# EPFL-VILAB/omnidata

Measured on AMD Instinct MI355X. Metric: images/sec (384x384) DPT-Hybrid surface-normal inference, higher is better.
Workload: dtype bf16; 1 GPU; DPT-Hybrid-384 normal, batch 32/GPU, bf16, 1xMI355X (BASELINE.json configs[1]); batch_per_gpu=32, global_batch=32, parallelism=replicas x1 (no collective in the loop), ranks_seen=1, inflight=1

## Files before the change

### omnidata_amd/csrc/attention.hip

```cpp
#include "common.h"
#include "kernels.h"

namespace dptx {

constexpr int ATT_D = 64;
constexpr int ATT_KT = 64;
constexpr int ATT_K_BYTES = ATT_KT * 128;
constexpr int ATT_V_BYTES = ATT_D * 128;
constexpr int ATT_STAGE = ATT_K_BYTES + ATT_V_BYTES;

__device__ __forceinline__ uint4 lds_read16(const char* p) {
  const u32x4_t v = *(const u32x4_t*)p;
  return uint4{v.x, v.y, v.z, v.w};
}

template <int DT, int PL>
__global__ __launch_bounds__(256, 2) void attention_kernel(const uint16_t* __restrict__ qkv, uint16_t* __restrict__ out,
                                                           int S, int H, int BH, long long plane) {
  extern __shared__ __attribute__((aligned(16))) char smem[];
  constexpr int STAGE = ATT_STAGE * PL;
  const int tid = threadIdx.x, lane = tid & 63, wave = tid >> 6;
  const int lr = lane & 31, lh = lane >> 5;
  const int bh = (int)blockIdx.x % BH, qblk = (int)blockIdx.x / BH;
  const int head = bh % H, b = bh / H;
  const int ld = 3 * H * ATT_D;
  const long long row0 = (long long)b * S;
  const uint16_t* qbase = qkv + head * ATT_D;
  const uint16_t* kbase = qkv + H * ATT_D + head * ATT_D;
  const uint16_t* vbase = qkv + 2 * H * ATT_D + head * ATT_D;

  const int q = qblk * 128 + wave * 32 + lr;
  const int qc = q < S ? q : S - 1;
  const bool wave_active = qblk * 128 + wave * 32 < S;
  uint4 qf[4], ql[4];
#pragma unroll
  for (int ks = 0; ks < 4; ++ks) {
    qf[ks] = *(const uint4*)(qbase + (row0 + qc) * ld + ks * 16 + lh * 8);
    if (PL == 2) ql[ks] = *(const uint4*)(qbase + plane + (row0 + qc) * ld + ks * 16 + lh * 8);
  }

  const u32x4_t zero4 = {0u, 0u, 0u, 0u};
#if defined(__HIP_DEVICE_COMPILE__)
  const int qkv_bytes = (int)((long long)(BH / H) * S * ld * 2);
  const __amdgpu_buffer_rsrc_t rsrc0 = __builtin_amdgcn_make_buffer_rsrc(const_cast<uint16_t*>(qkv), 0, qkv_bytes, 0x00020000);
  const __amdgpu_buffer_rsrc_t rsrc1 = __builtin_amdgcn_make_buffer_rsrc(const_cast<uint16_t*>(qkv) + (PL == 2 ? plane : 0), 0, qkv_bytes, 0x00020000);
  auto dma_kv = [&](int T, int buf) {
#pragma unroll
    for (int pc = 0; pc < 2; ++pc) {
      const int row = (wave * 2 + pc) * 8 + (lane >> 3);
      const int key = 1 + T * ATT_KT + row;
      const bool ok = key < S;
      const unsigned rowoff = (unsigned)((row0 + key) * ld + head * ATT_D);
      const unsigned koff = ok ? (rowoff + H * ATT_D + (((lane & 7) ^ ((row >> 1) & 7)) << 3)) * 2u : 0x80000000u;
      const unsigned voff = ok ? (rowoff + 2 * H * ATT_D + (((lane & 7) ^ (4 * ((row >> 1) & 1))) << 3)) * 2u : 0x80000000u;
      char* dst = smem + buf * STAGE + (wave * 2 + pc) * 1024;
      __builtin_amdgcn_raw_ptr_buffer_load_lds(rsrc0, (__attribute__((address_space(3))) void*)dst, 16, koff, 0, 0, 0);
      __builtin_amdgcn_raw_ptr_buffer_load_lds(rsrc0, (__attribute__((address_space(3))) void*)(dst + ATT_K_BYTES), 16, voff, 0, 0, 0);
      if (PL == 2) {
        __builtin_amdgcn_raw_ptr_buffer_load_lds(rsrc1, (__attribute__((address_space(3))) void*)(dst + ATT_STAGE), 16, koff, 0, 0, 0);
        __builtin_amdgcn_raw_ptr_buffer_load_lds(rsrc1, (__attribute__((address_space(3))) void*)(dst + ATT_STAGE + ATT_K_BYTES), 16, voff, 0, 0, 0);
      }
    }
  };
  const int lq = lane & 15, g16 = (lane >> 4) & 1;
  int va[2];
#pragma unroll
  for (int dt = 0; dt < 2; ++dt)
    va[dt] = (4 * lh + (lq >> 2)) * 128 + (((dt ^ ((lq >> 3) & 1)) * 4 + 2 * g16 + ((lq & 3) >> 1)) << 4) + (lq & 1) * 8;
  typedef short s16x4_t __attribute__((ext_vector_type(4)));
  typedef __attribute__((address_space(3))) s16x4_t* lds_s16x4_p;
  auto read_vt = [&](const char* vtile, int dt, int i) -> uint4 {
    const __attribute__((address_space(3))) char* vb = (const __attribute__((address_space(3))) char*)vtile + va[dt] + i * 2048;
    const s16x4_t r0_ = __builtin_amdgcn_ds_read_tr16_b64_v4i16((lds_s16x4_p)vb);
    const s16x4_t r1_ = __builtin_amdgcn_ds_read_tr16_b64_v4i16((lds_s16x4_p)(vb + 1024));
    const uint2 u0 = __builtin_bit_cast(uint2, r0_), u1 = __builtin_bit_cast(uint2, r1_);
    return uint4{u0.x, u0.y, u1.x, u1.y};
  };
#else
  auto dma_kv = [&](int, int) {};
  auto read_vt = [&](const char*, int, int) -> uint4 { return uint4{0u, 0u, 0u, 0u}; };
#endif

  const int ntiles = (S - 1 + ATT_KT - 1) / ATT_KT;
  if (ntiles > 0) dma_kv(0, 0);

  const float cexp = 0.125f * 1.4426950408889634f;
  f32x16_t o[2];
  float m_run, l_run;
  {
    float part = 0.f;
#pragma unroll
    for (int ks = 0; ks < 4; ++ks) {
      float qv[8], kv[8];
      u32x4_t qh = {qf[ks].x, qf[ks].y, qf[ks].z, qf[ks].w}, qlo = zero4;
      if (PL == 2) qlo = u32x4_t{ql[ks].x, ql[ks].y, ql[ks].z, ql[ks].w};
      unpack8x<DT, PL>(qh, qlo, qv);
      const u32x4_t kh = *(const u32x4_t*)(kbase + row0 * ld + ks * 16 + lh * 8);
      u32x4_t klo = zero4;
      if (PL == 2) klo = *(const u32x4_t*)(kbase + plane + row0 * ld + ks * 16 + lh * 8);
      unpack8x<DT, PL>(kh, klo, kv);
#pragma unroll
      for (int e = 0; e < 8; ++e) part = fmaf(qv[e], kv[e], part);
    }
    m_run = part + __shfl_xor(part, 32, 64);
    l_run = lh == 0 ? 1.f : 0.f;
#pragma unroll
    for (int dt = 0; dt < 2; ++dt)
#pragma unroll
      for (int g = 0; g < 4; ++g) {
        const int d = dt * 32 + 8 * g + 4 * lh;
        const uint2 vh = *(const uint2*)(vbase + row0 * ld + d);
        float v4[4] = {T16<DT>::tof((uint16_t)(vh.x & 0xffffu)), T16<DT>::tof((uint16_t)(vh.x >> 16)),
                       T16<DT>::tof((uint16_t)(vh.y & 0xffffu)), T16<DT>::tof((uint16_t)(vh.y >> 16))};
        if (PL == 2) {
          const uint2 vl = *(const uint2*)(vbase + plane + row0 * ld + d);
          v4[0] += T16<DT>::tof((uint16_t)(vl.x & 0xffffu)); v4[1] += T16<DT>::tof((uint16_t)(vl.x >> 16));
          v4[2] += T16<DT>::tof((uint16_t)(vl.y & 0xffffu)); v4[3] += T16<DT>::tof((uint16_t)(vl.y >> 16));
        }
#pragma unroll
        for (int e = 0; e < 4; ++e) o[dt][4 * g + e] = v4[e];
      }
  }

  asm volatile("s_waitcnt vmcnt(0)" ::: "memory");
  __syncthreads();
  for (int t = 0; t < ntiles; ++t) {
    const bool more = (t + 1) < ntiles;
    if (more) dma_kv(t + 1, (t + 1) & 1);
    const char* sk = smem + (t & 1) * STAGE;
    const char* sv = sk + ATT_K_BYTES;
    if (wave_active) {
      f32x16_t s0, s1;
#pragma unroll
      for (int r = 0; r < 16; ++r) { s0[r] = 0.f; s1[r] = 0.f; }
#pragma unroll
      for (int ks = 0; ks < 4; ++ks) {
        const int chunk = 2 * ks + lh;
        const int koff0 = lr * 128 + ((chunk ^ ((lr >> 1) & 7)) << 4);
        const int koff1 = koff0 + 32 * 128;
        const uint4 kf0 = lds_read16(sk + koff0), kf1 = lds_read16(sk + koff1);
        if (PL == 2) {
          const uint4 kl0 = lds_read16(sk + ATT_STAGE + koff0), kl1 = lds_read16(sk + ATT_STAGE + koff1);
          s0 = T16<DT>::mfma32(kl0, qf[ks], s0);
          s1 = T16<DT>::mfma32(kl1, qf[ks], s1);
          s0 = T16<DT>::mfma32(kf0, ql[ks], s0);
          s1 = T16<DT>::mfma32(kf1, ql[ks], s1);
        }
        s0 = T16<DT>::mfma32(kf0, qf[ks], s0);
        s1 = T16<DT>::mfma32(kf1, qf[ks], s1);
      }
      const int key0 = 1 + t * ATT_KT + 4 * lh;
      if (key0 + 32 + 28 + 3 >= S) {
#pragma unroll
        for (int r = 0; r < 16; ++r) {
          if (key0 + (r & 3) + 8 * (r >> 2) >= S) s0[r] = -1e30f;
          if (key0 + 32 + (r & 3) + 8 * (r >> 2) >= S) s1[r] = -1e30f;
        }
      }
      float mx = s0[0], mx1 = s1[0];
#pragma unroll
      for (int r = 1; r < 16; ++r) { mx = fmaxf(mx, s0[r]); mx1 = fmaxf(mx1, s1[r]); }
      mx = fmaxf(mx, mx1);
      mx = fmaxf(mx, __shfl_xor(mx, 32, 64));
      const float m_new = fmaxf(m_run, mx);
      const float alpha = __builtin_amdgcn_exp2f((m_run - m_new) * cexp);
      const bool grew = m_new > m_run;
      m_run = m_new;
      const float mc = m_new * cexp;
      float pv0[16], pv1[16];
      float ps = 0.f;
#pragma unroll
      for (int r = 0; r < 16; ++r) {
        pv0[r] = __builtin_amdgcn_exp2f(fmaf(s0[r], cexp, -mc));
        pv1[r] = __builtin_amdgcn_exp2f(fmaf(s1[r], cexp, -mc));
        ps += pv0[r] + pv1[r];
      }
      l_run = l_run * alpha + ps;
      if (__any(grew)) {
#pragma unroll
        for (int r = 0; r < 16; ++r) { o[0][r] *= alpha; o[1][r] *= alpha; }
      }
      uint4 pf[4], pl2[4];
      pf[0] = pack8<DT>(pv0);
      pf[1] = pack8<DT>(pv0 + 8);
      pf[2] = pack8<DT>(pv1);
      pf[3] = pack8<DT>(pv1 + 8);
      if (PL == 2) {
        float ph[8];
#pragma unroll
        for (int i = 0; i < 4; ++i) {
          const float* src = (i < 2 ? pv0 : pv1) + (i & 1) * 8;
          unpack8<DT>(pf[i], ph);
#pragma unroll
          for (int r = 0; r < 8; ++r) ph[r] = src[r] - ph[r];
          pl2[i] = pack8<DT>(ph);
        }
      }
#pragma unroll
      for (int i = 0; i < 4; ++i) {
#pragma unroll
        for (int dt = 0; dt < 2; ++dt) {
          const uint4 vf = read_vt(sv, dt, i);
          if (PL == 2) {
            const uint4 vl = read_vt(sv + ATT_STAGE, dt, i);
            o[dt] = T16<DT>::mfma32(vl, pf[i], o[dt]);
            o[dt] = T16<DT>::mfma32(vf, pl2[i], o[dt]);
          }
          o[dt] = T16<DT>::mfma32(vf, pf[i], o[dt]);
        }
      }
    }
    asm volatile("s_waitcnt vmcnt(0)" ::: "memory");
    __syncthreads();
  }

  const float l_tot = l_run + __shfl_xor(l_run, 32, 64);
  const float inv = 1.0f / l_tot;
  if (q < S) {
    uint16_t* op = out + (row0 + q) * (long long)(H * ATT_D) + head * ATT_D;
#pragma unroll
    for (int dt = 0; dt < 2; ++dt)
#pragma unroll
      for (int g = 0; g < 4; ++g) {
        const float v0 = o[dt][4 * g] * inv, v1 = o[dt][4 * g + 1] * inv, v2 = o[dt][4 * g + 2] * inv, v3 = o[dt][4 * g + 3] * inv;
        uint2 w;
        w.x = T16<DT>::pack2(v0, v1);
        w.y = T16<DT>::pack2(v2, v3);
        *(uint2*)(op + dt * 32 + 8 * g + 4 * lh) = w;
        if (PL == 2) {
          uint2 l;
          l.x = T16<DT>::pack2(v0 - T16<DT>::tof((uint16_t)(w.x & 0xffffu)), v1 - T16<DT>::tof((uint16_t)(w.x >> 16)));
          l.y = T16<DT>::pack2(v2 - T16<DT>::tof((uint16_t)(w.y & 0xffffu)), v3 - T16<DT>::tof((uint16_t)(w.y >> 16)));
          *(uint2*)(op + plane + dt * 32 + 8 * g + 4 * lh) = l;
        }
      }
  }
}

hipError_t launch_attention(int mode, const void* qkv, void* out, int B, int S, int heads, Planes pl, hipStream_t stream) {
  const int BH = B * heads;
  if ((long long)B * S * 3 * heads * ATT_D * 2 >= (1ll << 31)) return hipErrorInvalidValue;
  dim3 grid(((S + 127) / 128) * BH);
  if (mode == MODE_BF16)
    hipLaunchKernelGGL((attention_kernel<DT_BF16, 1>), grid, dim3(256), 2 * ATT_STAGE, stream, (const uint16_t*)qkv, (uint16_t*)out, S, heads, BH, 0ll);
  else if (mode == MODE_FP16)
    hipLaunchKernelGGL((attention_kernel<DT_FP16, 1>), grid, dim3(256), 2 * ATT_STAGE, stream, (const uint16_t*)qkv, (uint16_t*)out, S, heads, BH, 0ll);
  else if (mode == MODE_BF16X3) {
    ensure_dyn_smem((const void*)attention_kernel<DT_BF16, 2>, 4 * ATT_STAGE);
    hipLaunchKernelGGL((attention_kernel<DT_BF16, 2>), grid, dim3(256), 4 * ATT_STAGE, stream, (const uint16_t*)qkv, (uint16_t*)out, S, heads, BH, pl.act);
  } else if (mode == MODE_FP16X3) {
    ensure_dyn_smem((const void*)attention_kernel<DT_FP16, 2>, 4 * ATT_STAGE);
    hipLaunchKernelGGL((attention_kernel<DT_FP16, 2>), grid, dim3(256), 4 * ATT_STAGE, stream, (const uint16_t*)qkv, (uint16_t*)out, S, heads, BH, pl.act);
  } else
    return hipErrorInvalidValue;
  return hipGetLastError();
}

}
```

### omnidata_amd/build.py

```python
from __future__ import annotations

import os
import subprocess
import sys

HERE = os.path.dirname(os.path.abspath(__file__))
CSRC = os.path.join(HERE, "csrc")
LIB = os.path.join(HERE, "libdptx.so")
SOURCES = ["gemm.hip", "gemm_fp16.hip", "gemm_fp16e.hip", "gemm_x3.hip", "gemm_x2.hip", "gemm_fp8.hip", "attention.hip", "norm.hip", "misc.hip", "stem.hip", "head.hip", "prepost.hip", "refocus.hip", "midas_loss.hip", "vnl_loss.hip", "normal_loss.hip", "eval_metrics.hip", "engine.hip", "ops.hip"]
HEADERS = ["common.h", "kernels.h", "gemm_impl.h", "select.h", os.path.join("..", "..", "include", "dptx.h")]
_NOPK = ["-Xclang", "-target-feature", "-Xclang", "-packed-fp32-ops"]
SOURCE_FLAGS = {src: list(_NOPK) for src in ("norm.hip", "misc.hip", "gemm.hip", "gemm_fp16.hip", "gemm_fp16e.hip", "gemm_x3.hip",
                                             "gemm_x2.hip", "gemm_fp8.hip", "refocus.hip",
                                             "midas_loss.hip", "vnl_loss.hip", "normal_loss.hip", "eval_metrics.hip")}
EXPERIMENT_HEADERS = []


def source_hash(extra_flags=()) -> str:
    import hashlib
    h = hashlib.sha256()
    for name in sorted(SOURCES + HEADERS + EXPERIMENT_HEADERS):
        path = os.path.join(CSRC, name)
        h.update(os.path.basename(name).encode() + b"\0")
        with open(path, "rb") as f:
            h.update(f.read())
    h.update(" ".join(extra_flags).encode())
    h.update(repr(sorted(SOURCE_FLAGS.items())).encode())
    return h.hexdigest()[:16]


def _newer(dst: str, srcs) -> bool:
    if not os.path.exists(dst):
        return False
    t = os.path.getmtime(dst)
    return all(os.path.getmtime(s) <= t for s in srcs)


def built_hash(suffix: str = "") -> str:
    path = os.path.join(CSRC, "build" + suffix, "engine.srchash")
    return open(path).read().strip() if os.path.exists(path) else ""


def build(force: bool = False, verbose: bool = False) -> str:
    import fcntl
    suffix = os.environ.get("DPTX_LIB_SUFFIX", "")
    objdir = os.path.join(CSRC, "build" + suffix)
    os.makedirs(objdir, exist_ok=True)
    with open(os.path.join(objdir, ".lock"), "w") as lock:
        fcntl.flock(lock, fcntl.LOCK_EX)
        try:
            return _build_locked(force, verbose, suffix, objdir)
        finally:
            fcntl.flock(lock, fcntl.LOCK_UN)


def _build_locked(force: bool, verbose: bool, suffix: str, objdir: str) -> str:
    hipcc = os.environ.get("HIPCC", "/opt/rocm/bin/hipcc")
    extra = os.environ.get("DPTX_CXXFLAGS", "").split()
    LIB = os.path.join(HERE, f"libdptx{suffix}.so")
    hdrs = [os.path.join(CSRC, h) for h in HEADERS + EXPERIMENT_HEADERS]
    src_hash = source_hash(extra)
    hash_file = os.path.join(objdir, "engine.srchash")
    old_hash = open(hash_file).read().strip() if os.path.exists(hash_file) else ""
    objs = []
    procs = []
    for src in SOURCES:
# ... 38 lines not shown
```

### omnidata_amd/csrc/gemm.hip

```cpp
#include "gemm_impl.h"

namespace dptx {

hipError_t launch_gemm_16(int dt, const GemmParams& p, hipStream_t stream) {
  return dt == DT_BF16 ? launch_dt<DT_BF16, 1>(p, stream) : launch_gemm_fp16(p, stream);
}

void gemm_params_dense(GemmParams& p, int M, int N, int K) {
  p = GemmParams{};
  p.M = M; p.N = N; p.K = K; p.ldw = K;
  p.a_rpi = M > 0 ? M : 1; p.Wout = p.a_rpi; p.Hin = 1; p.Win = p.a_rpi; p.Cin = K; p.a_pix_stride = K;
  p.a_img_stride = 0; p.a_off = 0; p.ksz = 1; p.stride = 1; p.pad_t = 0; p.pad_l = 0;
  p.c_rpi = 0x7fffffff; p.c_img_rows = 0; p.c_row_off = 0; p.ldc = N;
  p.a_bytes = (long long)M * K * 2;
}

void gemm_params_conv(GemmParams& p, int B, int Hin, int Win, int Cin, int Cout, int ksz, int stride, int pad_t, int pad_l,
                      int Hout, int Wout, int a_elem_bytes) {
  p = GemmParams{};
  p.M = B * Hout * Wout; p.N = Cout; p.K = ksz * ksz * Cin; p.ldw = p.K;
  p.a_rpi = Hout * Wout; p.Wout = Wout; p.Hin = Hin; p.Win = Win; p.Cin = Cin; p.a_pix_stride = Cin;
  p.a_img_stride = (long long)Hin * Win * Cin; p.a_off = 0; p.ksz = ksz; p.stride = stride; p.pad_t = pad_t; p.pad_l = pad_l;
  p.c_rpi = 0x7fffffff; p.c_img_rows = 0; p.c_row_off = 0; p.ldc = Cout;
  p.a_bytes = (long long)B * Hin * Win * Cin * a_elem_bytes;
  p.k_tap_fast = (ksz == 3 && Cin >= 512) ? 1 : 0;
}

static thread_local long long* g_trace = nullptr;
void gemm_set_trace(long long* dev_buf) { g_trace = dev_buf; }
static thread_local int g_debug_flags = 0;
void gemm_set_debug_flags(int flags) { g_debug_flags = flags; }
static thread_local float g_cu_share = 1.0f;
void gemm_set_cu_share(float share) { g_cu_share = share > 0.f && share <= 1.f ? share : 1.0f; }

hipError_t launch_gemm(int mode, const GemmParams& p0, hipStream_t stream) {
  GemmParams p = p0;
  p.trace = g_trace;
  p.debug_flags = g_debug_flags;
  if (p.cu_share <= 0.f) p.cu_share = g_cu_share;
  p.a_rpi_rcp = 1.0f / (float)(p.a_rpi > 0 ? p.a_rpi : 1);
  p.wout_rcp = 1.0f / (float)(p.Wout > 0 ? p.Wout : 1);
  if (p.gn_part != nullptr && (p.gn_hw % 32 != 0 || p.N % 32 != 0 || p.gn_cpg != p.N / 32 || p.gn_cpg < 2 || p.gn_cpg > 32 ||
                               (p.gn_cpg & (p.gn_cpg - 1)) != 0 || p.bias != nullptr || p.act != 0))
    return hipErrorInvalidValue;
  if (p.row_stats != nullptr && (p.N % 128 != 0 || p.stats_nblk != 8 || p.N / 128 > 8)) return hipErrorInvalidValue;
  if (p.ln_stats != nullptr && (p.R1 != nullptr || p.R2 != nullptr || p.bias_per_img || p.ln_colsum == nullptr || (p.ln_nblk != 6 && p.ln_nblk != 8) ||
                                p.c_rpi != 0x7fffffff || p.gn_part != nullptr))
    return hipErrorInvalidValue;
  if (mode == MODE_FP8) {
    if (p.K % 128 != 0 || p.Cin % 128 != 0 || p.M <= 0 || p.N % 32 != 0 || p.ldw < p.K || p.ldw % 16 != 0 || p.gn_part != nullptr)
      return hipErrorInvalidValue;
    return launch_gemm_fp8(p, stream);
  }
  if (p.K % BK != 0 || p.Cin % BK != 0 || p.M <= 0 || p.N % 32 != 0 || p.ldw < p.K || p.ldw % 8 != 0) return hipErrorInvalidValue;
  if (mode == MODE_BF16) return p.epi2 ? hipErrorInvalidValue : launch_gemm_16(DT_BF16, p, stream);
  if (mode == MODE_FP16) return p.epi2 ? launch_gemm_fp16e(p, stream) : launch_gemm_16(DT_FP16, p, stream);
  if (mode == MODE_BF16X3) return launch_gemm_x3(DT_BF16, p, stream);
  if (mode == MODE_FP16X3) return p.a_hi_only ? launch_gemm_x2(p, stream) : launch_gemm_x3(DT_FP16, p, stream);
  return hipErrorInvalidValue;
}

}
```

### omnidata_amd/csrc/gemm_impl.h

```cpp
#pragma once
#include <cstdlib>
#include <type_traits>

#include "common.h"
#include "kernels.h"

namespace dptx {

constexpr int BK = 64;

__device__ __forceinline__ int row_div(int m, int d, float rcp, bool big, int& rem) {
  if (big) {
    const int q = m / d;
    rem = m - q * d;
    return q;
  }
  int q = (int)((float)m * rcp);
  int r = m - q * d;
  if (r < 0) { --q; r += d; }
  if (r >= d) { ++q; r -= d; }
  rem = r;
  return q;
}

// ... 66 lines not shown
#pragma unroll
      for (int ks = 0; ks < HK; ++ks) {
#pragma unroll
        for (int i = 0; i < TM; ++i) {
          if (RELU_A) af[ks][i] = relu8(af[ks][i]);
#pragma unroll
          for (int j = 0; j < TN; ++j) acc[i][j] = T16<DT>::mfma32(af[ks][i], bf[ks][j], acc[i][j]);
        }
      }
      if (HK != BK / 16) __builtin_amdgcn_sched_barrier(0);
    }
    return;
  } else {
    u32x4_t af[2][TM], bf[2][TN], al[2][TM], bl[2][TN];
    auto read = [&](int s_, int ks) {
      const int chunk = 2 * ks + lh;
#pragma unroll
      for (int i = 0; i < TM; ++i) {
        const int row = wm * (TM * 32) + i * 32 + lr;
        const int off = row * 128 + ((chunk ^ ((row >> 1) & 7)) << 4);
        af[s_][i] = *(const u32x4_t*)(sa + off);
        if (XT == 3) al[s_][i] = *(const u32x4_t*)(sa + a_lo + off);
      }
#pragma unroll
      for (int j = 0; j < TN; ++j) {
        const int row = wn * (TN * 32) + j * 32 + lr;
        const int off = row * 128 + ((chunk ^ ((row >> 1) & 7)) << 4);
        bf[s_][j] = *(const u32x4_t*)(sb + off);
        bl[s_][j] = *(const u32x4_t*)(sb + b_lo + off);
      }
    };
    auto mma = [&](int s_) {
#pragma unroll
      for (int i = 0; i < TM; ++i) {
        if (RELU_A) {
          if (XT == 3) relu8_planes(af[s_][i], al[s_][i]);
          else af[s_][i] = relu8(af[s_][i]);
        }
#pragma unroll
        for (int j = 0; j < TN; ++j) {
          if (XT == 3) acc[i][j] = T16<DT>::mfma32(al[s_][i], bf[s_][j], acc[i][j]);
          acc[i][j] = T16<DT>::mfma32(af[s_][i], bl[s_][j], acc[i][j]);
          acc[i][j] = T16<DT>::mfma32(af[s_][i], bf[s_][j], acc[i][j]);
        }
      }
    };
    read(0, 0);
#pragma unroll
    for (int ks = 0; ks < BK / 16; ++ks) {
      if (ks + 1 < BK / 16) read((ks + 1) & 1, ks + 1);
      __builtin_amdgcn_sched_barrier(0);
      mma(ks & 1);
      __builtin_amdgcn_sched_barrier(0);
    }
  }
}

template <int DT, int BM, int BN, int TM, int TN, int PL = 1, int NT = 256, int SLABS = 1, bool WP = false>
__device__ __forceinline__ void epilogue(const GemmParams& p, char* smem, int m0, int n0, int wm, int wn, int lr, int lh,
                                         int tid, f32x16_t (&acc)[TM][TN], int row_pitch = 0, bool dma_in_flight = false,
                                         int trace_row = -1, const char* lds_ln = nullptr) {
  static_assert(SLABS == 1 || SLABS == TM, "one slab, or one per MFMA row tile");
  static_assert(!WP || (SLABS == TM && TN == 2), "wave-private staging: one 32 x 64 block per wave and slab");
  constexpr int CT_PITCH = WP ? 72 : BN + 4;
  constexpr int CT_ROWS = WP ? 32 : BM / SLABS;
  constexpr int NCH = WP ? 8 : BN / 8;
  constexpr int RPP = WP ? 8 : NT / NCH;
  constexpr int ITER = CT_ROWS / RPP;
  constexpr int WAVES_N = BN / (TN * 32);
  static_assert(CT_ROWS % RPP == 0, "rows per pass must divide the slab");
#ifdef DPTX_TRACE
#define DPTX_ESTAMP(SLOT)                                                                                          \
  do {                                                                                                             \
    if (p.trace != nullptr && blockIdx.x == 0 && tid == 0 && trace_row >= 0)                                       \
      p.trace[(48 + trace_row) * 4 + (SLOT)] = (long long)__builtin_readcyclecounter();                            \
  } while (0)
#else
#define DPTX_ESTAMP(SLOT) do { } while (0)
  (void)trace_row;
#endif
  DPTX_ESTAMP(0);
  float* ct = (float*)smem + (WP ? (wm * WAVES_N + wn) * (32 * CT_PITCH) : 0);
  const int cn = WP ? tid & 7 : tid % NCH;
  const int rr = WP ? (tid & 63) >> 3 : tid / NCH;
  const int n = n0 + (WP ? wn * (TN * 32) : 0) + cn * 8;

  if (p.gn_part != nullptr) {
    const int cpg = p.gn_cpg;
    const int cpg_sh = __builtin_ctz(cpg);
    int gn_hw = p.gn_hw;
    asm volatile("" : "+s"(gn_hw));
#pragma unroll
    for (int i = 0; i < TM; ++i) {
      const int mb = m0 + (wm * TM + i) * 32;
      const int img = mb / gn_hw;
      const int blk = (mb - img * gn_hw) >> 5;
#pragma unroll
      for (int j = 0; j < TN; ++j) {
        float sm = 0.f, sq = 0.f;
#pragma unroll
        for (int r = 0; r < 16; ++r) { const float v = acc[i][j][r]; sm += v; sq = fmaf(v, v, sq); }
        sm += __shfl_xor(sm, 32, 64);
        sq += __shfl_xor(sq, 32, 64);
        for (int o = 1; o < cpg; o <<= 1) { sm += __shfl_xor(sm, o, 64); sq += __shfl_xor(sq, o, 64); }
        if (lh == 0 && (lr & (cpg - 1)) == 0 && mb < p.M) {
          const int g = (n0 + (wn * TN + j) * 32 + lr) >> cpg_sh;
          float2* dst = (float2*)p.gn_part + ((long long)img * p.gn_blocks + blk) * 32 + g;
          *dst = make_float2(sm, sq);
        }
      }
    }
  }

  float bias_c[8];
#pragma unroll
  for (int e = 0; e < 8; ++e) bias_c[e] = 0.f;
  if (p.bias != nullptr && !p.bias_per_img) {
    const float4 b0 = *(const float4*)(p.bias + n), b1 = *(const float4*)(p.bias + n + 4);
    bias_c[0] = b0.x; bias_c[1] = b0.y; bias_c[2] = b0.z; bias_c[3] = b0.w;
    bias_c[4] = b1.x; bias_c[5] = b1.y; bias_c[6] = b1.z; bias_c[7] = b1.w;
  }
  float osc[8];
  if (p.out_scale != 0.f) {
#pragma unroll
    for (int e = 0; e < 8; ++e) osc[e] = p.out_scale;
    if (p.out_scale_v != nullptr) {
      const float4 s0 = *(const float4*)(p.out_scale_v + n), s1 = *(const float4*)(p.out_scale_v + n + 4);
      osc[0] *= s0.x; osc[1] *= s0.y; osc[2] *= s0.z; osc[3] *= s0.w;
      osc[4] *= s1.x; osc[5] *= s1.y; osc[6] *= s1.z; osc[7] *= s1.w;
    }
  }
  const bool remap = p.c_rpi != 0x7fffffff;
  int c_rpi = p.c_rpi;
  asm volatile("" : "+s"(c_rpi));
  float2* lnrow = (float2*)(smem + (WP ? (size_t)(NT / 64) * 32 * CT_PITCH * 4 : (size_t)CT_ROWS * CT_PITCH * 4));
  if (p.ln_stats != nullptr) {
    const bool all8 = p.ln_nblk == 8;
    for (int r = tid; r < BM; r += NT) {
      int R = r;
      if (row_pitch) R = (R >> 5) * row_pitch + (R & 31);
      int m = m0 + R;
      m = m < p.M ? m : m0;
      const float4* st = lds_ln != nullptr ? (const float4*)(lds_ln + r * 64) : (const float4*)(p.ln_stats + (long long)m * 16);
      const float4 r0 = st[0], r1_ = st[1], r2_ = st[2], r3_ = st[3];
      const float sm = (r0.x + r0.z) + (r1_.x + r1_.z) + ((r2_.x + r2_.z) + (all8 ? r3_.x + r3_.z : 0.f));
      const float sq = (r0.y + r0.w) + (r1_.y + r1_.w) + ((r2_.y + r2_.w) + (all8 ? r3_.y + r3_.w : 0.f));
      lnrow[r] = ln_mu_rstd(sm, sq, p.ln_inv_dim, p.ln_eps);
    }
    if (WP) __syncthreads();
  }
  DPTX_ESTAMP(1);
  constexpr int GR_ = SLABS > 1 ? 2 : (ITER < 4 ? ITER : 4);
  static_assert(ITER % GR_ == 0, "row groups");

  auto body = [&](auto r1m_, auto r2m_, auto bpi_, auto lnf_) {
    constexpr int R1M = decltype(r1m_)::value, R2M = decltype(r2m_)::value, BPI = decltype(bpi_)::value;
    constexpr bool LNF = decltype(lnf_)::value != 0;
    constexpr int GR = (SLABS > 1 && (R1M < 0 || (PL == 2 && R1M != 0 && R2M != 0))) ? 1 : GR_;
    constexpr int NGR = ITER / GR;
    float ln_c[8];
    if (LNF) {
      const float4 c0 = *(const float4*)(p.ln_colsum + n), c1 = *(const float4*)(p.ln_colsum + n + 4);
      ln_c[0] = c0.x; ln_c[1] = c0.y; ln_c[2] = c0.z; ln_c[3] = c0.w;
      ln_c[4] = c1.x; ln_c[5] = c1.y; ln_c[6] = c1.z; ln_c[7] = c1.w;
    }
// ... 1219 lines not shown
```

### omnidata_amd/csrc/kernels.h

```cpp
#pragma once
#include <hip/hip_runtime.h>
#include <stdint.h>

#include "common.h"

namespace dptx {

void ensure_dyn_smem(const void* kernel, size_t bytes);

struct GemmParams {
  const void* A;
  const void* W;
  void* C;
  const float* bias;
  const void* R1;
  const void* R2;
  int M, N, K;
  int ldw;
  int a_rpi, Wout, Hin, Win, Cin, a_pix_stride;
  long long a_img_stride, a_off;
  long long a_bytes;
  int ksz, stride, pad_t, pad_l;
  int c_rpi, c_img_rows, c_row_off, ldc;
  int r2_bcast;
  int bias_per_img;
  int act;
  int a_relu;
  int a_fp32;
  int c_fp32, r1_fp32, r2_fp32;
  Planes planes;
  int epi2, c_hi_only, r1_hi_only, r2_hi_only;
  int a_hi_only;
  int xcd_m, xcd_n;
  float cu_share;
  float pad0;
  int k_tap_fast;
  float* gn_part;
  int gn_hw, gn_blocks, gn_cpg;
  void* C8;
  int q_relu;
  float out_scale, q_scale;
  const float* out_scale_v;
  void* C16;
  float* row_stats;
  int stats_nblk;
  const float* ln_stats;
  const float* ln_colsum;
  int ln_nblk;
  float ln_eps, ln_inv_dim;
  long long* trace;
  int debug_flags;
  float a_rpi_rcp, wout_rcp;
};

void gemm_params_dense(GemmParams& p, int M, int N, int K);
void gemm_params_conv(GemmParams& p, int B, int Hin, int Win, int Cin, int Cout, int ksz, int stride, int pad_t, int pad_l,
                      int Hout, int Wout, int a_elem_bytes);
hipError_t launch_gemm(int dtype, const GemmParams& p, hipStream_t stream);
void gemm_set_trace(long long* dev_buf);
void gemm_set_debug_flags(int flags);
void gemm_set_cu_share(float share);

hipError_t launch_attention(int mode, const void* qkv, void* out, int B, int S, int heads, Planes pl, hipStream_t stream);

hipError_t launch_layernorm(int mode, const float* x, const float* gamma, const float* beta, void* y,
                            int M, int C, float eps, Planes pl, hipStream_t stream);

struct GnParams {
  const void* X; void* Y;
  const float* gamma; const float* beta;
  float* partial;
  const void* R;
  const float* r_gamma; const float* r_beta; const float* r_partial;
  int B, HW, C, relu;
  float eps;
  int nrec;
};
int gn_chunks(int HW, int C);
hipError_t launch_gn_stats(int mode, const void* X, float* partial, int B, int HW, int C, Planes pl, hipStream_t stream);
hipError_t launch_gn_apply(int mode, const GnParams& p, Planes pl, hipStream_t stream);
hipError_t launch_gn_relu_maxpool(int mode, const void* X, void* Y, const float* gamma, const float* beta,
                                  const float* partial, int B, int H, int W, int C, float eps, Planes pl, hipStream_t stream);

hipError_t launch_stem_conv(int mode, const void* x, int io, const void* Wt, void* y, int B, int H, int W, Planes pl,
                            hipStream_t stream);

hipError_t launch_upsample2x(int mode, const void* X, void* Y, int B, int H, int W, int C, Planes pl, hipStream_t stream,
                             void* Y8 = nullptr, float q_scale = 1.0f, bool out_hi_only = false);
hipError_t launch_amax(int mode, const void* X, size_t n, int relu, unsigned* amax_bits, hipStream_t stream);

hipError_t launch_nonfinite_scan(int mode, const void* X, size_t n, unsigned* flag, hipStream_t stream);

hipError_t launch_checksum(const void* p, size_t bytes, unsigned long long* out, hipStream_t stream);
hipError_t launch_spin(long long ticks_100mhz, hipStream_t stream);

hipError_t launch_head_out(int mode, const void* X, const float* w, const float* b, void* y, int io, int B, int HW,
                           int Cout, int relu, Planes pl, hipStream_t stream);

hipError_t launch_head_tail(int mode, const void* H0, const void* W2, const float* b2, const float* w4, const float* b4,
                            void* y, int io, int B, int Hs, int Ws, int C, int relu_out, hipStream_t stream, Planes pl = Planes{0, 0});
hipError_t launch_pos_resize(const float* src, float* dst, int g_old, int gh, int gw, int C, hipStream_t stream);
hipError_t launch_cls_rows(int mode, const float* cls, const float* pos, float* X, int B, int S, int C, void* X16, float* stats,
                           hipStream_t stream, void* X8 = nullptr, float q_scale = 1.0f);

hipError_t launch_readout_cls(int mode, const float* x, long long x_stride, const void* W, int ldw, int w_off,
                              const float* bias, float* out, int B, int N, int K, Planes pl, hipStream_t stream, int x16 = 0);
hipError_t launch_cast_f32(int mode, const float* src, void* dst, size_t n, Planes pl, hipStream_t stream);

hipError_t launch_patchify16(int mode, const void* x, int io, void* P, int B, int H, int W, Planes pl, hipStream_t stream);
hipError_t launch_depth_to_space(int mode, const void* G, void* Y, int B, int h, int w, int k, int C, Planes pl, hipStream_t stream);

hipError_t launch_to_f32(int mode, const void* src, float* dst, size_t n, Planes pl, hipStream_t stream);

// ... 2 lines not shown
```

Before: 2678 images/s.

## Remap attention blocks by head groups, hoist DMA offsets, use permlane32 swaps

Changes the block-to-(head,qblock) mapping so consecutive blocks cover groups of 8 heads across all query blocks, which improves K/V reuse in L2. Per-lane K/V buffer offsets are precomputed once and the tile offset is passed through soffset, which removes address arithmetic from the loop. Cross-half reductions use permlane32_swap instead of shuffles. The output epilogue swaps halves so each lane writes 16-byte stores instead of 8-byte ones. The grid is padded to a multiple of 8 heads with an early exit, and the unsigned 32-bit soffset math relies on the existing size guard.

Result: no change. 2691 images/s (median of 6 runs) (+0.5%).

```diff
diff --git a/omnidata_amd/csrc/attention.hip b/omnidata_amd/csrc/attention.hip
--- a/omnidata_amd/csrc/attention.hip
+++ b/omnidata_amd/csrc/attention.hip
@@ -9,19 +9,48 @@
 constexpr int ATT_V_BYTES = ATT_D * 128;
 constexpr int ATT_STAGE = ATT_K_BYTES + ATT_V_BYTES;
 
+__device__ __forceinline__ void swap_halves(unsigned& a, unsigned& b) {
+#if defined(__HIP_DEVICE_COMPILE__)
+  const auto r = __builtin_amdgcn_permlane32_swap(a, b, false, false);
+  a = r[0];
+  b = r[1];
+#endif
+}
+__device__ __forceinline__ float max_both_halves(float x) {
+  unsigned a = __float_as_uint(x), b = a;
+  swap_halves(a, b);
+  return fmaxf(__uint_as_float(a), __uint_as_float(b));
+}
+
+__device__ __forceinline__ float sum_both_halves(float x) {
+  unsigned a = __float_as_uint(x), b = a;
+  swap_halves(a, b);
+  return __uint_as_float(a) + __uint_as_float(b);
+}
+
 __device__ __forceinline__ uint4 lds_read16(const char* p) {
   const u32x4_t v = *(const u32x4_t*)p;
   return uint4{v.x, v.y, v.z, v.w};
 }
+
+__host__ __device__ __forceinline__ void att_block_map(int id, int nq, int& pair, int& qblk) {
+  const int j = id >> 3;
+  pair = (j / nq) * 8 + (id & 7);
+  qblk = j % nq;
+}
+inline int att_grid(int S, int BH) { return 8 * ((BH + 7) / 8) * ((S + 127) / 128); }
 
 template <int DT, int PL>
 __global__ __launch_bounds__(256, 2) void attention_kernel(const uint16_t* __restrict__ qkv, uint16_t* __restrict__ out,
                                                            int S, int H, int BH, long long plane) {
   extern __shared__ __attribute__((aligned(16))) char smem[];
   constexpr int STAGE = ATT_STAGE * PL;
-  const int tid = threadIdx.x, lane = tid & 63, wave = tid >> 6;
+  const int tid = threadIdx.x, lane = tid & 63;
+  const int wave = __builtin_amdgcn_readfirstlane(tid >> 6);
   const int lr = lane & 31, lh = lane >> 5;
-  const int bh = (int)blockIdx.x % BH, qblk = (int)blockIdx.x / BH;
+  int bh, qblk;
+  att_block_map((int)blockIdx.x, (S + 127) >> 7, bh, qblk);
+  if (bh >= BH) return;
   const int head = bh % H, b = bh / H;
   const int ld = 3 * H * ATT_D;
   const long long row0 = (long long)b * S;
@@ -44,21 +73,29 @@
   const int qkv_bytes = (int)((long long)(BH / H) * S * ld * 2);
   const __amdgpu_buffer_rsrc_t rsrc0 = __builtin_amdgcn_make_buffer_rsrc(const_cast<uint16_t*>(qkv), 0, qkv_bytes, 0x00020000);
   const __amdgpu_buffer_rsrc_t rsrc1 = __builtin_amdgcn_make_buffer_rsrc(const_cast<uint16_t*>(qkv) + (PL == 2 ? plane : 0), 0, qkv_bytes, 0x00020000);
+  unsigned koff0[2], voff0[2];
+  int krow[2];
+#pragma unroll
+  for (int pc = 0; pc < 2; ++pc) {
+    const int row = (wave * 2 + pc) * 8 + (lane >> 3);
+    const unsigned rowoff = (unsigned)((row0 + 1 + row) * ld + head * ATT_D);
+    krow[pc] = row;
+    koff0[pc] = (rowoff + H * ATT_D + (((lane & 7) ^ ((row >> 1) & 7)) << 3)) * 2u;
+    voff0[pc] = (rowoff + 2 * H * ATT_D + (((lane & 7) ^ (4 * ((row >> 1) & 1))) << 3)) * 2u;
+  }
   auto dma_kv = [&](int T, int buf) {
+    const int soff = T * ATT_KT * ld * 2;
+    const int left = S - 1 - T * ATT_KT;
 #pragma unroll
     for (int pc = 0; pc < 2; ++pc) {
-      const int row = (wave * 2 + pc) * 8 + (lane >> 3);
-      const int key = 1 + T * ATT_KT + row;
-      const bool ok = key < S;
-      const unsigned rowoff = (unsigned)((row0 + key) * ld + head * ATT_D);
-      const unsigned koff = ok ? (rowoff + H * ATT_D + (((lane & 7) ^ ((row >> 1) & 7)) << 3)) * 2u : 0x80000000u;
-      const unsigned voff = ok ? (rowoff + 2 * H * ATT_D + (((lane & 7) ^ (4 * ((row >> 1) & 1))) << 3)) * 2u : 0x80000000u;
+      const bool ok = krow[pc] < left;
+      const unsigned koff = ok ? koff0[pc] : 0x80000000u, voff = ok ? voff0[pc] : 0x80000000u;
       char* dst = smem + buf * STAGE + (wave * 2 + pc) * 1024;
-      __builtin_amdgcn_raw_ptr_buffer_load_lds(rsrc0, (__attribute__((address_space(3))) void*)dst, 16, koff, 0, 0, 0);
-      __builtin_amdgcn_raw_ptr_buffer_load_lds(rsrc0, (__attribute__((address_space(3))) void*)(dst + ATT_K_BYTES), 16, voff, 0, 0, 0);
+      __builtin_amdgcn_raw_ptr_buffer_load_lds(rsrc0, (__attribute__((address_space(3))) void*)dst, 16, koff, soff, 0, 0);
+      __builtin_amdgcn_raw_ptr_buffer_load_lds(rsrc0, (__attribute__((address_space(3))) void*)(dst + ATT_K_BYTES), 16, voff, soff, 0, 0);
       if (PL == 2) {
-        __builtin_amdgcn_raw_ptr_buffer_load_lds(rsrc1, (__attribute__((address_space(3))) void*)(dst + ATT_STAGE), 16, koff, 0, 0, 0);
-        __builtin_amdgcn_raw_ptr_buffer_load_lds(rsrc1, (__attribute__((address_space(3))) void*)(dst + ATT_STAGE + ATT_K_BYTES), 16, voff, 0, 0, 0);
+        __builtin_amdgcn_raw_ptr_buffer_load_lds(rsrc1, (__attribute__((address_space(3))) void*)(dst + ATT_STAGE), 16, koff, soff, 0, 0);
+        __builtin_amdgcn_raw_ptr_buffer_load_lds(rsrc1, (__attribute__((address_space(3))) void*)(dst + ATT_STAGE + ATT_K_BYTES), 16, voff, soff, 0, 0);
       }
     }
   };
@@ -102,7 +139,7 @@
 #pragma unroll
       for (int e = 0; e < 8; ++e) part = fmaf(qv[e], kv[e], part);
     }
-    m_run = part + __shfl_xor(part, 32, 64);
+    m_run = sum_both_halves(part);
     l_run = lh == 0 ? 1.f : 0.f;
 #pragma unroll
     for (int dt = 0; dt < 2; ++dt)
@@ -161,7 +198,7 @@
 #pragma unroll
       for (int r = 1; r < 16; ++r) { mx = fmaxf(mx, s0[r]); mx1 = fmaxf(mx1, s1[r]); }
       mx = fmaxf(mx, mx1);
-      mx = fmaxf(mx, __shfl_xor(mx, 32, 64));
+      mx = max_both_halves(mx);
       const float m_new = fmaxf(m_run, mx);
       const float alpha = __builtin_amdgcn_exp2f((m_run - m_new) * cexp);
       const bool grew = m_new > m_run;
@@ -214,33 +251,48 @@
     __syncthreads();
   }
 
-  const float l_tot = l_run + __shfl_xor(l_run, 32, 64);
+  const float l_tot = sum_both_halves(l_run);
   const float inv = 1.0f / l_tot;
+  uint4 sth[4], stl[4];
+#pragma unroll
+  for (int dt = 0; dt < 2; ++dt)
+#pragma unroll
+    for (int g = 0; g < 4; g += 2) {
+      uint2 w[2], l[2];
+#pragma unroll
+      for (int j = 0; j < 2; ++j) {
+        const int r = 4 * (g + j);
+        const float v0 = o[dt][r] * inv, v1 = o[dt][r + 1] * inv, v2 = o[dt][r + 2] * inv, v3 = o[dt][r + 3] * inv;
+        w[j].x = T16<DT>::pack2(v0, v1);
+        w[j].y = T16<DT>::pack2(v2, v3);
+        if (PL == 2) {
+          l[j].x = T16<DT>::pack2(v0 - T16<DT>::tof((uint16_t)(w[j].x & 0xffffu)), v1 - T16<DT>::tof((uint16_t)(w[j].x >> 16)));
+          l[j].y = T16<DT>::pack2(v2 - T16<DT>::tof((uint16_t)(w[j].y & 0xffffu)), v3 - T16<DT>::tof((uint16_t)(w[j].y >> 16)));
+        }
+      }
+      swap_halves(w[0].x, w[1].x);
+      swap_halves(w[0].y, w[1].y);
+      sth[dt * 2 + g / 2] = uint4{w[0].x, w[0].y, w[1].x, w[1].y};
+      if (PL == 2) {
+        swap_halves(l[0].x, l[1].x);
+        swap_halves(l[0].y, l[1].y);
+        stl[dt * 2 + g / 2] = uint4{l[0].x, l[0].y, l[1].x, l[1].y};
+      }
+    }
   if (q < S) {
-    uint16_t* op = out + (row0 + q) * (long long)(H * ATT_D) + head * ATT_D;
-#pragma unroll
-    for (int dt = 0; dt < 2; ++dt)
-#pragma unroll
-      for (int g = 0; g < 4; ++g) {
-        const float v0 = o[dt][4 * g] * inv, v1 = o[dt][4 * g + 1] * inv, v2 = o[dt][4 * g + 2] * inv, v3 = o[dt][4 * g + 3] * inv;
-        uint2 w;
-        w.x = T16<DT>::pack2(v0, v1);
-        w.y = T16<DT>::pack2(v2, v3);
-        *(uint2*)(op + dt * 32 + 8 * g + 4 * lh) = w;
-        if (PL == 2) {
-          uint2 l;
-          l.x = T16<DT>::pack2(v0 - T16<DT>::tof((uint16_t)(w.x & 0xffffu)), v1 - T16<DT>::tof((uint16_t)(w.x >> 16)));
-          l.y = T16<DT>::pack2(v2 - T16<DT>::tof((uint16_t)(w.y & 0xffffu)), v3 - T16<DT>::tof((uint16_t)(w.y >> 16)));
-          *(uint2*)(op + plane + dt * 32 + 8 * g + 4 * lh) = l;
-        }
-      }
+    uint16_t* op = out + (row0 + q) * (long long)(H * ATT_D) + head * ATT_D + 8 * lh;
+#pragma unroll
+    for (int i = 0; i < 4; ++i) {
+      *(uint4*)(op + 16 * i) = sth[i];
+      if (PL == 2) *(uint4*)(op + plane + 16 * i) = stl[i];
+    }
   }
 }
 
 hipError_t launch_attention(int mode, const void* qkv, void* out, int B, int S, int heads, Planes pl, hipStream_t stream) {
   const int BH = B * heads;
   if ((long long)B * S * 3 * heads * ATT_D * 2 >= (1ll << 31)) return hipErrorInvalidValue;
-  dim3 grid(((S + 127) / 128) * BH);
+  dim3 grid(att_grid(S, BH));
   if (mode == MODE_BF16)
     hipLaunchKernelGGL((attention_kernel<DT_BF16, 1>), grid, dim3(256), 2 * ATT_STAGE, stream, (const uint16_t*)qkv, (uint16_t*)out, S, heads, BH, 0ll);
   else if (mode == MODE_FP16)
```

## Add persistent weight-resident kernel for small-K 1x1 convolutions

Applied to the files above, without the earlier changes.

Adds a specialized streaming kernel for 1x1 convs with K of 64/128/256. It keeps the whole weight panel resident in LDS, gives each wave its own 32-row A tiles with prefetch, and stages output through LDS for coalesced stores. It is routed in automatically for a whitelist of shapes in the ResNet backbone of DPT-Hybrid. The aim is to cut the per-tile weight reloads and K-loop overhead that the generic GEMM pays on these thin-K convolutions. The GN stats epilogue is factored into a shared helper so the new kernel can reuse it.

Result: faster. 2616 images/s before, 2658 images/s after (median of 6 runs) (+1.6%).

```diff
diff --git a/omnidata_amd/build.py b/omnidata_amd/build.py
--- a/omnidata_amd/build.py
+++ b/omnidata_amd/build.py
@@ -7,11 +7,11 @@
 HERE = os.path.dirname(os.path.abspath(__file__))
 CSRC = os.path.join(HERE, "csrc")
 LIB = os.path.join(HERE, "libdptx.so")
-SOURCES = ["gemm.hip", "gemm_fp16.hip", "gemm_fp16e.hip", "gemm_x3.hip", "gemm_x2.hip", "gemm_fp8.hip", "attention.hip", "norm.hip", "misc.hip", "stem.hip", "head.hip", "prepost.hip", "refocus.hip", "midas_loss.hip", "vnl_loss.hip", "normal_loss.hip", "eval_metrics.hip", "engine.hip", "ops.hip"]
+SOURCES = ["gemm.hip", "gemm_fp16.hip", "gemm_fp16e.hip", "gemm_x3.hip", "gemm_x2.hip", "gemm_fp8.hip", "conv1x1.hip", "attention.hip", "norm.hip", "misc.hip", "stem.hip", "head.hip", "prepost.hip", "refocus.hip", "midas_loss.hip", "vnl_loss.hip", "normal_loss.hip", "eval_metrics.hip", "engine.hip", "ops.hip"]
 HEADERS = ["common.h", "kernels.h", "gemm_impl.h", "select.h", os.path.join("..", "..", "include", "dptx.h")]
 _NOPK = ["-Xclang", "-target-feature", "-Xclang", "-packed-fp32-ops"]
 SOURCE_FLAGS = {src: list(_NOPK) for src in ("norm.hip", "misc.hip", "gemm.hip", "gemm_fp16.hip", "gemm_fp16e.hip", "gemm_x3.hip",
-                                             "gemm_x2.hip", "gemm_fp8.hip", "refocus.hip",
+                                             "gemm_x2.hip", "gemm_fp8.hip", "conv1x1.hip", "refocus.hip",
                                              "midas_loss.hip", "vnl_loss.hip", "normal_loss.hip", "eval_metrics.hip")}
 EXPERIMENT_HEADERS = []
 
diff --git a/omnidata_amd/csrc/conv1x1.hip b/omnidata_amd/csrc/conv1x1.hip
--- /dev/null
+++ b/omnidata_amd/csrc/conv1x1.hip
@@ -0,0 +1,209 @@
+#include "gemm_impl.h"
+
+namespace dptx {
+
+constexpr int C1_STG_PITCH = 144;
+constexpr int C1_STG_WAVE = 16 * C1_STG_PITCH;
+constexpr int C1_WAVES = 4;
+
+template <int KT, int BN>
+constexpr size_t conv1x1_smem_bytes() {
+  return (size_t)KT * BN * 128 + (size_t)C1_WAVES * KT * 32 * 128 + (size_t)C1_WAVES * C1_STG_WAVE;
+}
+
+template <int DT, int KT, int BN>
+__global__ __launch_bounds__(64 * C1_WAVES, KT <= 2 ? 2 : 1) void conv1x1_stream_kernel(const GemmParams p) {
+#if defined(__HIP_DEVICE_COMPILE__)
+  constexpr int NSUB = BN / 64;
+  constexpr int KS = KT * 4;
+  constexpr int W_BYTES = KT * BN * 128;
+  constexpr int A_WAVE = KT * 32 * 128;
+  extern __shared__ __attribute__((aligned(16))) char smem[];
+
+  const int tid = threadIdx.x;
+  const int lane = tid & 63;
+  const int wave = __builtin_amdgcn_readfirstlane(tid >> 6);
+  const int lr = lane & 31, lh = lane >> 5;
+
+  const int npan = p.N / BN;
+  const int x = (int)blockIdx.x & 7, l = (int)blockIdx.x >> 3;
+  const int n0 = (l % npan) * BN;
+  const int slots = ((int)gridDim.x / npan) * C1_WAVES;
+  const int rb_total = (p.M + 31) >> 5;
+  int rb = ((l / npan) * 8 + x) * C1_WAVES + wave;
+
+  const int w_bytes = (int)((long long)p.N * p.ldw * 2);
+  const __amdgpu_buffer_rsrc_t rsrcA = __builtin_amdgcn_make_buffer_rsrc(const_cast<void*>(p.A), 0, (int)p.a_bytes, 0x00020000);
+  const __amdgpu_buffer_rsrc_t rsrcW = __builtin_amdgcn_make_buffer_rsrc(const_cast<void*>(p.W), 0, w_bytes, 0x00020000);
+
+  char* const sw = smem;
+  char* const sa = smem + W_BYTES + wave * A_WAVE;
+  char* const stg = smem + W_BYTES + C1_WAVES * A_WAVE + wave * C1_STG_WAVE;
+
+  const int kc = lane & 7, r0 = lane >> 3;
+  auto issue_a = [&](int rblk) {
+#pragma unroll
+    for (int i = 0; i < 4; ++i) {
+      const int row = r0 + 8 * i;
+      const int m = rblk * 32 + row;
+      const bool ok = m < p.M;
+      const int mm = ok ? m : 0;
+      int rem, ox;
+      const int img = row_div(mm, p.a_rpi, p.a_rpi_rcp, false, rem);
+      const int oy = row_div(rem, p.Wout, p.wout_rcp, false, ox);
+      const int iy = oy * p.stride - p.pad_t, ix = ox * p.stride - p.pad_l;
+      const bool valid = ok && ((unsigned)iy < (unsigned)p.Hin) && ((unsigned)ix < (unsigned)p.Win);
+      const long long e = (long long)img * p.a_img_stride + p.a_off + ((long long)iy * p.Win + ix) * p.a_pix_stride +
+                          (kc ^ ((row >> 1) & 7)) * 8;
+      const unsigned base = (unsigned)(e * 2);
+#pragma unroll
+      for (int kt = 0; kt < KT; ++kt) {
+        const unsigned vo = valid ? base + kt * 128 : OOB;
+        __builtin_amdgcn_raw_ptr_buffer_load_lds(rsrcA, (__attribute__((address_space(3))) void*)(sa + kt * 4096 + i * 1024), 16, vo,
+                                                 0, 0, 0);
+      }
+    }
+  };
+
+  if (rb < rb_total) issue_a(rb);
+  for (int idx = wave; idx < KT * (BN / 8); idx += C1_WAVES) {
+    const int kt = idx / (BN / 8), rg = idx - kt * (BN / 8);
+    const int row = rg * 8 + r0;
+    const unsigned vo = (unsigned)(((long long)(n0 + row) * p.ldw + kt * 64 + (kc ^ ((row >> 1) & 7)) * 8) * 2);
+    __builtin_amdgcn_raw_ptr_buffer_load_lds(rsrcW, (__attribute__((address_space(3))) void*)(sw + kt * (BN * 128) + rg * 1024), 16, vo,
+                                             0, 0, 0);
+  }
+  float bias_c[NSUB][2];
+#pragma unroll
+  for (int s = 0; s < NSUB; ++s)
+#pragma unroll
+    for (int j = 0; j < 2; ++j) bias_c[s][j] = p.bias != nullptr ? p.bias[n0 + s * 64 + j * 32 + lr] : 0.f;
+  asm volatile("s_waitcnt vmcnt(0)" ::: "memory");
+  __syncthreads();
+
+  const int swz = (lr >> 1) & 7;
+  const unsigned sel = (lr & 1) ? 0x03020706u : 0x05040100u;
+  const int cn = lane & 7, rr = lane >> 3;
+
+  for (; rb < rb_total; rb += slots) {
+    const int m0 = rb * 32;
+    u32x4_t af[KS];
+#pragma unroll
+    for (int ks = 0; ks < KS; ++ks)
+      af[ks] = *(const u32x4_t*)(sa + (ks >> 2) * 4096 + lr * 128 + (((2 * (ks & 3) + lh) ^ swz) << 4));
+    asm volatile("s_waitcnt lgkmcnt(0)" ::: "memory");
+    const bool prefetch = rb + slots < rb_total;
+    if (prefetch) issue_a(rb + slots);
+
+#pragma unroll
+    for (int s = 0; s < NSUB; ++s) {
+      f32x16_t acc[1][2];
+#pragma unroll
+      for (int j = 0; j < 2; ++j)
+#pragma unroll
+        for (int r = 0; r < 16; ++r) acc[0][j][r] = 0.f;
+#pragma unroll
+      for (int kt = 0; kt < KT; ++kt) {
+        u32x4_t bf[4][2];
+#pragma unroll
+        for (int q = 0; q < 4; ++q)
+#pragma unroll
+          for (int j = 0; j < 2; ++j)
+            bf[q][j] = *(const u32x4_t*)(sw + kt * (BN * 128) + (s * 64 + j * 32 + lr) * 128 + (((2 * q + lh) ^ swz) << 4));
+        __builtin_amdgcn_sched_barrier(0);
+#pragma unroll
+        for (int q = 0; q < 4; ++q)
+#pragma unroll
+          for (int j = 0; j < 2; ++j) acc[0][j] = T16<DT>::mfma32(af[kt * 4 + q], bf[q][j], acc[0][j]);
+      }
+      if (s == 0) {
+        __builtin_amdgcn_sched_barrier(0);
+        asm volatile("s_waitcnt vmcnt(0)" ::: "memory");
+      }
+      if (p.gn_part != nullptr) gn_records<1, 2>(p, m0, n0 + s * 64, 0, 0, lr, lh, acc);
+
+#pragma unroll
+      for (int h = 0; h < 2; ++h) {
+        asm volatile("" ::: "memory");
+        __builtin_amdgcn_wave_barrier();
+#pragma unroll
+        for (int j = 0; j < 2; ++j)
+#pragma unroll
+          for (int t = 0; t < 4; ++t) {
+            float v0 = acc[0][j][8 * h + 2 * t] + bias_c[s][j], v1 = acc[0][j][8 * h + 2 * t + 1] + bias_c[s][j];
+            if (p.act == 1) { v0 = fmaxf(v0, 0.f); v1 = fmaxf(v1, 0.f); }
+            const uint32_t own = T16<DT>::pack2(v0, v1);
+            const uint32_t nb = (uint32_t)__builtin_amdgcn_update_dpp(0, (int)own, 0xB1, 0xf, 0xf, false);
+            const uint32_t o = __builtin_amdgcn_perm(nb, own, sel);
+            const int rl = ((2 * t) & 3) + (lr & 1) + 8 * (t >> 1) + 4 * lh;
+            *(uint32_t*)(stg + rl * C1_STG_PITCH + (j * 32 + (lr & ~1)) * 2) = o;
+          }
+        asm volatile("" ::: "memory");
+        __builtin_amdgcn_wave_barrier();
+#pragma unroll
+        for (int pp = 0; pp < 2; ++pp) {
+          const int rl = rr + 8 * pp;
+          const u32x4_t d = *(const u32x4_t*)(stg + rl * C1_STG_PITCH + cn * 16);
+          const int m = m0 + 16 * h + rl;
+          if (m < p.M) *(u32x4_t*)((uint16_t*)p.C + (long long)(p.c_row_off + m) * p.ldc + (n0 + s * 64 + cn * 8)) = d;
+        }
+      }
+    }
+  }
+#endif
+}
+
+bool conv1x1_stream_eligible(int mode, const GemmParams& p) {
+  if (mode != MODE_BF16 && mode != MODE_FP16) return false;
+  if (p.ksz != 1 || p.pad_t != 0 || p.pad_l != 0 || (p.stride != 1 && p.stride != 2)) return false;
+  if (p.K != p.Cin || (p.K != 64 && p.K != 128 && p.K != 256) || p.N % 64 != 0) return false;
+  if (p.a_fp32 || p.c_fp32 || p.epi2 || p.a_relu || p.R1 != nullptr || p.R2 != nullptr || p.bias_per_img) return false;
+  if (p.c_rpi != 0x7fffffff || p.C8 != nullptr || p.C16 != nullptr || p.out_scale != 0.f) return false;
+  if (p.row_stats != nullptr || p.ln_stats != nullptr || (p.act != 0 && p.act != 1)) return false;
+  if (p.ldc % 8 != 0 || p.a_pix_stride % 8 != 0 || p.a_off % 8 != 0 || p.a_img_stride % 8 != 0) return false;
+  if (p.a_bytes <= 0 || p.a_bytes >= (1ll << 31) || (long long)p.N * p.ldw * 2 >= (1ll << 31) || p.M >= (1 << 23)) return false;
+  return true;
+}
+
+bool conv1x1_stream_adopted(const GemmParams& p) {
+  if (p.stride != 1) return false;
+  if (p.K == 64) return p.N == 256 || p.N == 64;
+  if (p.K == 128) return p.N == 512;
+  if (p.K == 256) return p.N == 64 || p.N == 128 || (p.N == 256 && p.a_rpi >= 48 * 48);
+  return false;
+}
+
+template <int DT, int KT, int BN>
+static hipError_t launch_c1(const GemmParams& p, hipStream_t stream) {
+  constexpr size_t smem = conv1x1_smem_bytes<KT, BN>();
+  static_assert(smem <= 160 * 1024 && (KT > 2 || 2 * smem <= 160 * 1024), "two blocks per CU at K <= 128");
+  const int npan = p.N / BN;
+  const int rb_total = (p.M + 31) / 32;
+  const int want = (rb_total + C1_WAVES - 1) / C1_WAVES;
+  int cap = (KT <= 2 ? 512 : 256) / npan;
+  if (cap < 8) cap = 8;
+  int groups = want < cap ? want : cap;
+  groups = (groups + 7) / 8 * 8;
+  auto k = conv1x1_stream_kernel<DT, KT, BN>;
+  set_smem_attr(k, smem);
+  hipLaunchKernelGGL(k, dim3(groups * npan), dim3(64 * C1_WAVES), smem, stream, p);
+  return hipGetLastError();
+}
+
+template <int DT>
+static hipError_t launch_c1_dt(const GemmParams& p, hipStream_t stream) {
+  if (p.K == 64) {
+    if (p.N % 256 == 0) return launch_c1<DT, 1, 256>(p, stream);
+    if (p.N % 128 == 0) return launch_c1<DT, 1, 128>(p, stream);
+    return launch_c1<DT, 1, 64>(p, stream);
+  }
+  if (p.K == 128) return p.N % 128 == 0 ? launch_c1<DT, 2, 128>(p, stream) : launch_c1<DT, 2, 64>(p, stream);
+  return p.N % 128 == 0 ? launch_c1<DT, 4, 128>(p, stream) : launch_c1<DT, 4, 64>(p, stream);
+}
+
+hipError_t launch_conv1x1_stream(int mode, const GemmParams& p, hipStream_t stream) {
+  if (!conv1x1_stream_eligible(mode, p)) return hipErrorInvalidValue;
+  return mode == MODE_BF16 ? launch_c1_dt<DT_BF16>(p, stream) : launch_c1_dt<DT_FP16>(p, stream);
+}
+
+}
diff --git a/omnidata_amd/csrc/gemm.hip b/omnidata_amd/csrc/gemm.hip
--- a/omnidata_amd/csrc/gemm.hip
+++ b/omnidata_amd/csrc/gemm.hip
@@ -53,6 +53,8 @@
     return launch_gemm_fp8(p, stream);
   }
   if (p.K % BK != 0 || p.Cin % BK != 0 || p.M <= 0 || p.N % 32 != 0 || p.ldw < p.K || p.ldw % 8 != 0) return hipErrorInvalidValue;
+  if (!(p.debug_flags & 8) && conv1x1_stream_eligible(mode, p) && ((p.debug_flags & 16) || conv1x1_stream_adopted(p)))
+    return launch_conv1x1_stream(mode, p, stream);
   if (mode == MODE_BF16) return p.epi2 ? hipErrorInvalidValue : launch_gemm_16(DT_BF16, p, stream);
   if (mode == MODE_FP16) return p.epi2 ? launch_gemm_fp16e(p, stream) : launch_gemm_16(DT_FP16, p, stream);
   if (mode == MODE_BF16X3) return launch_gemm_x3(DT_BF16, p, stream);
diff --git a/omnidata_amd/csrc/gemm_impl.h b/omnidata_amd/csrc/gemm_impl.h
--- a/omnidata_amd/csrc/gemm_impl.h
+++ b/omnidata_amd/csrc/gemm_impl.h
@@ -142,6 +142,35 @@
       __builtin_amdgcn_sched_barrier(0);
       mma(ks & 1);
       __builtin_amdgcn_sched_barrier(0);
+    }
+  }
+}
+
+template <int TM, int TN>
+__device__ __forceinline__ void gn_records(const GemmParams& p, int m0, int n0, int wm, int wn, int lr, int lh,
+                                           f32x16_t (&acc)[TM][TN]) {
+  const int cpg = p.gn_cpg;
+  const int cpg_sh = __builtin_ctz(cpg);
+  int gn_hw = p.gn_hw;
+  asm volatile("" : "+s"(gn_hw));
+#pragma unroll
+  for (int i = 0; i < TM; ++i) {
+    const int mb = m0 + (wm * TM + i) * 32;
+    const int img = mb / gn_hw;
+    const int blk = (mb - img * gn_hw) >> 5;
+#pragma unroll
+    for (int j = 0; j < TN; ++j) {
+      float sm = 0.f, sq = 0.f;
+#pragma unroll
+      for (int r = 0; r < 16; ++r) { const float v = acc[i][j][r]; sm += v; sq = fmaf(v, v, sq); }
+      sm += __shfl_xor(sm, 32, 64);
+      sq += __shfl_xor(sq, 32, 64);
+      for (int o = 1; o < cpg; o <<= 1) { sm += __shfl_xor(sm, o, 64); sq += __shfl_xor(sq, o, 64); }
+      if (lh == 0 && (lr & (cpg - 1)) == 0 && mb < p.M) {
+        const int g = (n0 + (wn * TN + j) * 32 + lr) >> cpg_sh;
+        float2* dst = (float2*)p.gn_part + ((long long)img * p.gn_blocks + blk) * 32 + g;
+        *dst = make_float2(sm, sq);
+      }
     }
   }
 }
@@ -175,32 +204,7 @@
   const int rr = WP ? (tid & 63) >> 3 : tid / NCH;
   const int n = n0 + (WP ? wn * (TN * 32) : 0) + cn * 8;
 
-  if (p.gn_part != nullptr) {
-    const int cpg = p.gn_cpg;
-    const int cpg_sh = __builtin_ctz(cpg);
-    int gn_hw = p.gn_hw;
-    asm volatile("" : "+s"(gn_hw));
-#pragma unroll
-    for (int i = 0; i < TM; ++i) {
-      const int mb = m0 + (wm * TM + i) * 32;
-      const int img = mb / gn_hw;
-      const int blk = (mb - img * gn_hw) >> 5;
-#pragma unroll
-      for (int j = 0; j < TN; ++j) {
-        float sm = 0.f, sq = 0.f;
-#pragma unroll
-        for (int r = 0; r < 16; ++r) { const float v = acc[i][j][r]; sm += v; sq = fmaf(v, v, sq); }
-        sm += __shfl_xor(sm, 32, 64);
-        sq += __shfl_xor(sq, 32, 64);
-        for (int o = 1; o < cpg; o <<= 1) { sm += __shfl_xor(sm, o, 64); sq += __shfl_xor(sq, o, 64); }
-        if (lh == 0 && (lr & (cpg - 1)) == 0 && mb < p.M) {
-          const int g = (n0 + (wn * TN + j) * 32 + lr) >> cpg_sh;
-          float2* dst = (float2*)p.gn_part + ((long long)img * p.gn_blocks + blk) * 32 + g;
-          *dst = make_float2(sm, sq);
-        }
-      }
-    }
-  }
+  if (p.gn_part != nullptr) gn_records<TM, TN>(p, m0, n0, wm, wn, lr, lh, acc);
 
   float bias_c[8];
 #pragma unroll
diff --git a/omnidata_amd/csrc/kernels.h b/omnidata_amd/csrc/kernels.h
--- a/omnidata_amd/csrc/kernels.h
+++ b/omnidata_amd/csrc/kernels.h
@@ -59,6 +59,9 @@
 hipError_t launch_gemm(int dtype, const GemmParams& p, hipStream_t stream);
 void gemm_set_trace(long long* dev_buf);
 void gemm_set_debug_flags(int flags);
+bool conv1x1_stream_eligible(int mode, const GemmParams& p);
+bool conv1x1_stream_adopted(const GemmParams& p);
+hipError_t launch_conv1x1_stream(int mode, const GemmParams& p, hipStream_t stream);
 void gemm_set_cu_share(float share);
 
 hipError_t launch_attention(int mode, const void* qkv, void* out, int B, int S, int heads, Planes pl, hipStream_t stream);
```
